# carlostojal/NDT-Net

Hardware: AMD Instinct MI355X
Metric: clouds/sec NDT preprocess+PointNet fwd, 100k pts->1000 NDs, batch=16 (higher is better)
Workload: dtype f64 NDT; PointNet fp32-accurate split-bf16x3 (6 products) on 11 per-point layers, fp32 MFMA on the K=16 first layers and the TNet / seg-bias FC layers

## Files before the change

### include/ndnet_pointnet.h

```cpp
#ifndef NDNET_POINTNET_H_
#define NDNET_POINTNET_H_
#include <stdint.h>

#ifdef __cplusplus
extern "C" {
#endif

#define NDNET_PN_MAX_LAYERS 5

typedef struct ndnet_pn_layer {
  const float* w;
  int64_t w_cloud_stride;
  const float* bias;
  int64_t bias_cloud_stride;
  int32_t K, N;
  int32_t relu;
  int32_t prec;
  int32_t fuse_next;
} ndnet_pn_layer;

typedef struct ndnet_pn_chain {
  const float* x;
  int32_t x_ld;
  int32_t in_cols;
// ... 26 lines not shown
} ndnet_pn_chain;

int ndnet_pn_chain_run(const ndnet_pn_chain *args, int batch, void *stream);
int ndnet_pn_chain_run_t32(const ndnet_pn_chain *args, int batch, void *stream);

int ndnet_pn_debug_stamps(unsigned long long *host, int wgs);
int ndnet_pn_debug_stamps_clear(void);

int ndnet_pn_fc_run(const float *in, int ld_in, const float *W, const float *bias, float *out, int ld_out,
                    int batch, int K, int N, int relu, void *stream);
int ndnet_pn_fc_mfma_run(const float *in, int ld_in, const float *Wf, const float *bias, float *out, int ld_out,
                         int batch, int K, int N, int relu, void *stream);
int ndnet_pn_fc_mfma_bias_run(const float *in, int ld_in, const float *Wf, const float *bias, int bias_ld, float *out,
                              int ld_out, int batch, int K, int N, int relu, void *stream);
int ndnet_pn_cls_head_run(const float *in, int ld_in, const float *Wf, const float *bias, float *probs,
                          int ld_probs, float *logits, int ld_logits, int batch, int K, int N, int out_cols,
                          float *clear, int64_t clear_count, void *stream);
#define NDNET_FOLD_WT 0
#define NDNET_FOLD_FRAG 1
#define NDNET_FOLD_FRAG6 2
#define NDNET_FOLD_ROWS 3
#define NDNET_FOLD_BASIS 4
#define NDNET_FOLD_BIAS 5
typedef struct ndnet_pn_fold_job {
  const float *w;
  const float *bias;
  const float *gamma, *beta, *mean, *var;
  void *out;
  int32_t kind;
  int32_t N, K;
  int32_t ld, k0;
  int32_t Kp, Np;
  int32_t eye;
  float eps;
  int32_t reserved;
  int64_t block0;
} ndnet_pn_fold_job;
int ndnet_pn_fold_prepare(ndnet_pn_fold_job *host_jobs, int num_jobs, int64_t *num_blocks);
int ndnet_pn_fold_run(const ndnet_pn_fold_job *device_jobs, int num_jobs, int64_t num_blocks, void *stream);

int ndnet_pn_head3_run(const float *h2, int ld_h, const float *W3, const float *b3, const float *basis,
                       float *t1, float *w1f, int batch, int K, int kin, int nout, void *stream);

int ndnet_pn_fold_t2_run(const float *w1f, int w1_stride, const float *b1, const float *t2, int t2_ld, float *outf,
                         float *outb, int batch, void *stream);

int ndnet_pn_fold_seg_run(const float *w1f, int w1_stride, const float *b1, const float *t2, int t2_ld, float *outf,
                          float *outb, const float *s1aT, const float *s1b, int N2, float *wd, int64_t wd_stride,
                          float *bd, int64_t bd_stride, int batch, void *stream);

int ndnet_pn_pool12_run(const float *x, int x_ld, int num_points, const float *w0f, int64_t w0_stride,
                        const float *b0, int64_t b0_stride, const float *w_mid, const float *b_mid,
                        const float *w_tail, const float *b_tail, int F, int Fp, float *gmax, int gmax_ld,
                        int batch, void *stream);

#ifdef __cplusplus
}
#endif

#endif
```

### ndt-net_amd/csrc/pointnet_kernels.hip

```cpp
#include <hip/hip_runtime.h>
#include <math.h>
#include <stdint.h>
#include <stdio.h>
#include <stdlib.h>

#include "../../include/ndnet_pointnet.h"

namespace {

#ifndef NDNET_PN_TILE
#define NDNET_PN_TILE 64
#endif
constexpr int kP = NDNET_PN_TILE;
#ifndef NDNET_PN_WAVES
#define NDNET_PN_WAVES (NDNET_PN_TILE / 4)
#endif
constexpr int kWaves = NDNET_PN_WAVES;
constexpr int kThreads = 64 * kWaves;
constexpr int kRowBlocks = kP / 16;
static_assert(kP == 64 || kP == 32, "64- or 32-point tiles");
constexpr int kFuseNC = 64;
constexpr int kPadF = 8;
constexpr int kPadB = 16;
#ifndef NDNET_PN_PLANE_SWZ
// ... 1355 lines not shown
    else bd[(int64_t)b * bd_stride + col] = (float)(acc + (double)sb);
  }
}

#if NDNET_PN_TILE == 64
typedef double f64x4 __attribute__((ext_vector_type(4)));
constexpr int kP12Waves = 16;
constexpr int kP12Pre = 4;
constexpr int kP12Pitch = 130;

__device__ inline void p12_rows(const float* __restrict__ xb, int x_ld, int n, int tile, int kq, int cl, float (&v)[3]) {
  const int p = min(16 * tile + cl, n - 1);
  const float* r = xb + (int64_t)p * x_ld + kq;
#pragma unroll
  for (int s = 0; s < 3; s++) v[s] = r[4 * s];
}

__device__ inline void p12_clean(int n, int tile, int cl, float (&v)[3]) {
  const bool in = 16 * tile + cl < n;
#pragma unroll
  for (int s = 0; s < 3; s++) v[s] = (in & (fabsf(v[s]) < INFINITY)) ? v[s] : NAN;
}

__global__ void __launch_bounds__(kP12Waves * 64) k_pn_pool12(
    const float* __restrict__ x, int x_ld, int n, const float* __restrict__ w0f, int64_t w0_stride,
    const float* __restrict__ b0, int64_t b0_stride, const float* __restrict__ w_mid,
    const float* __restrict__ b_mid, const float* __restrict__ w_tail, const float* __restrict__ b_tail, int Fp,
    float* __restrict__ gmax, int gmax_ld) {
  __shared__ double s_m[13 * kP12Pitch];
  __shared__ float s_wc[13 * 64];
  __shared__ float s_red[kP12Waves * 64];
  const int b = blockIdx.y, c0 = 64 * blockIdx.x;
  const int lane = threadIdx.x & 63, kq = lane >> 4, cl = lane & 15;
  const int wave = __builtin_amdgcn_readfirstlane((int)threadIdx.x >> 6);
  const int tiles = (n + 15) >> 4;
  const float* xb = x + (int64_t)b * n * x_ld;

  float xp[kP12Pre][3];
#pragma unroll
  for (int i = 0; i < kP12Pre; i++) p12_rows(xb, x_ld, n, wave + kP12Waves * i, kq, cl, xp[i]);
  float tw[32];

  if (wave < 8) {
    const float* wb = w0f + (int64_t)b * w0_stride;
    const float* bb = b0 + (int64_t)b * b0_stride;
    float a[16], bw[16];
#pragma unroll
    for (int ks = 0; ks < 16; ks++) {
      const int i = 4 * ks + kq;
      const float* src = cl < 12 ? wb + ((((i >> 4) * 64 + ((cl >> 2) & 3) * 16 + (i & 15)) << 2) + (cl & 3)) : bb + i;
      a[ks] = *src;
      bw[ks] = w_mid[i * 128 + 16 * wave + cl];
    }
#pragma unroll
    for (int ks = 0; ks < 16; ks++) a[ks] = cl < 13 ? a[ks] : 0.0f;
    f64x4 acc0 = {0.0, 0.0, 0.0, 0.0}, acc1 = {0.0, 0.0, 0.0, 0.0};
#pragma unroll
    for (int ks = 0; ks < 16; ks += 2) {
      acc0 = __builtin_amdgcn_mfma_f64_16x16x4f64((double)a[ks], (double)bw[ks], acc0, 0, 0, 0);
      acc1 = __builtin_amdgcn_mfma_f64_16x16x4f64((double)a[ks + 1], (double)bw[ks + 1], acc1, 0, 0, 0);
    }
#pragma unroll
    for (int q = 0; q < 4; q++) {
      const int row = kq + 4 * q, col = 16 * wave + cl;
      double v = acc0[q] + acc1[q];
// ... 1 lines not shown
      if (row < 13) s_m[row * kP12Pitch + col] = v;
    }
  } else if (wave < 12) {
    const int tc = min(c0 + 16 * (wave - 8) + cl, Fp - 1);
#pragma unroll
    for (int ks = 0; ks < 32; ks++) tw[ks] = w_tail[(int64_t)(4 * ks + kq) * Fp + tc];
  }
  __syncthreads();
  if (wave >= 8 && wave < 12) {
    f64x4 acc0 = {0.0, 0.0, 0.0, 0.0}, acc1 = {0.0, 0.0, 0.0, 0.0};
#pragma unroll
    for (int ks = 0; ks < 32; ks += 2) {
      const double a0 = s_m[min(cl, 12) * kP12Pitch + 4 * ks + kq], a1 = s_m[min(cl, 12) * kP12Pitch + 4 * ks + 4 + kq];
      acc0 = __builtin_amdgcn_mfma_f64_16x16x4f64(cl < 13 ? a0 : 0.0, (double)tw[ks], acc0, 0, 0, 0);
      acc1 = __builtin_amdgcn_mfma_f64_16x16x4f64(cl < 13 ? a1 : 0.0, (double)tw[ks + 1], acc1, 0, 0, 0);
    }
#pragma unroll
    for (int q = 0; q < 4; q++) {
      const int row = kq + 4 * q, col = 16 * (wave - 8) + cl;
      double v = acc0[q] + acc1[q];
      if (row == 12) v += (double)b_tail[min(c0 + col, Fp - 1)];
      if (row < 13) s_wc[row * 64 + col] = (float)v;
    }
  }
  __syncthreads();

  float wc[4][3];
#pragma unroll
  for (int cb = 0; cb < 4; cb++)
#pragma unroll
    for (int s = 0; s < 3; s++) wc[cb][s] = s_wc[(4 * s + kq) * 64 + 16 * cb + cl];
  float m[4][4];
#pragma unroll
  for (int cb = 0; cb < 4; cb++)
#pragma unroll
    for (int r = 0; r < 4; r++) m[cb][r] = -INFINITY;
  auto tile = [&](int t, float (&xv)[3]) {
    p12_clean(n, t, cl, xv);
    f32x4 acc[4];
#pragma unroll
    for (int cb = 0; cb < 4; cb++) acc[cb] = f32x4{0.f, 0.f, 0.f, 0.f};
#pragma unroll
    for (int s = 0; s < 3; s++)
#pragma unroll
      for (int cb = 0; cb < 4; cb++) acc[cb] = __builtin_amdgcn_mfma_f32_16x16x4f32(wc[cb][s], xv[s], acc[cb], 0, 0, 0);
#pragma unroll
// ... 101 lines not shown
constexpr int kFoldThreads = 256;

__device__ inline uint16_t fold_bf16(float x) {
  uint32_t u = __float_as_uint(x);
  if ((u & 0x7fffffffu) > 0x7f800000u) return (uint16_t)((u >> 16) | 0x40u);
  return (uint16_t)((u + 0x7fffu + ((u >> 16) & 1u)) >> 16);
}

__device__ inline float fold_w(const ndnet_pn_fold_job& J, int n, int k) {
#pragma clang fp contract(off)
  if (n >= J.N || k >= J.K) return 0.0f;
  const float w = J.w[(int64_t)n * J.ld + J.k0 + k];
  if (!J.gamma) return w;
  return w * (J.gamma[n] / sqrtf(J.var[n] + J.eps));
}

__host__ __device__ inline int64_t fold_units(const ndnet_pn_fold_job& J) {
  switch (J.kind) {
    case NDNET_FOLD_WT: return (int64_t)J.Kp * J.Np;
    case NDNET_FOLD_FRAG: return (int64_t)J.Kp * J.Np / 4;
    case NDNET_FOLD_FRAG6: return (int64_t)J.Kp * J.Np / 8;
    case NDNET_FOLD_ROWS: return (int64_t)J.N * J.K;
    case NDNET_FOLD_BASIS: return (int64_t)9 * J.K * J.N;
    default: return J.Np;
  }
}

__global__ void __launch_bounds__(kFoldThreads) k_pn_fold(const ndnet_pn_fold_job* __restrict__ jobs, int num_jobs) {
#pragma clang fp contract(off)
  int j = 0;
  for (int i = 1; i < num_jobs; i++)
    if (jobs[i].block0 <= (int64_t)blockIdx.x) j = i;
  const ndnet_pn_fold_job J = jobs[j];
  const int64_t u = ((int64_t)blockIdx.x - J.block0) * kFoldThreads + threadIdx.x;
  if (u >= fold_units(J)) return;
  switch (J.kind) {
    case NDNET_FOLD_WT: {
      const int n = (int)(u % J.Np), k = (int)(u / J.Np);
      static_cast<float*>(J.out)[u] = fold_w(J, n, k);
      break;
    }
    case NDNET_FOLD_FRAG: {
      const int kgs = J.Kp / 16;
      const int cl = (int)(u % 16), kq = (int)(u / 16 % 4), kg = (int)(u / 64 % kgs), cb = (int)(u / (64 * kgs));
      const int k = 16 * kg + 4 * kq, n = 16 * cb + cl;
      f32x4 v = {fold_w(J, n, k), fold_w(J, n, k + 1), fold_w(J, n, k + 2), fold_w(J, n, k + 3)};
      reinterpret_cast<f32x4*>(J.out)[u] = v;
      break;
    }
    case NDNET_FOLD_FRAG6: {
      const int kgs = J.Kp / 32;
      const int cl = (int)(u % 16), kq = (int)(u / 16 % 4), kg = (int)(u / 64 % kgs), cb = (int)(u / (64 * kgs));
      const int k = 32 * kg + 8 * kq, n = 16 * cb + cl;
      uint32_t p[3][4];
#pragma unroll
      for (int t = 0; t < 8; t += 2) {
        uint16_t hv[2], mv[2], lv[2];
// ... 10 lines not shown
        p[2][t / 2] = lv[0] | ((uint32_t)lv[1] << 16);
      }
      const int64_t unit = u % 64 + (u / 64) * 192;
      uint4* o = reinterpret_cast<uint4*>(J.out);
#pragma unroll
      for (int pl = 0; pl < 3; pl++) o[unit + 64 * pl] = make_uint4(p[pl][0], p[pl][1], p[pl][2], p[pl][3]);
      break;
    }
    case NDNET_FOLD_ROWS: {
      const int n = (int)(u / J.K), k = (int)(u % J.K);
      static_cast<float*>(J.out)[u] = fold_w(J, n, k);
      break;
    }
    case NDNET_FOLD_BASIS: {
      const int n = (int)(u % J.N), r = (int)(u / J.N % J.K), ac = (int)(u / ((int64_t)J.N * J.K));
      const int a = ac / 3, c = ac % 3;
      float v = 0.0f;
      if (r < 3) {
        if (r == c) v = fold_w(J, n, a);
      } else if ((r - 3) / 3 == c) {
        v = fold_w(J, n, 3 + 3 * a + (r - 3) % 3);
      }
      static_cast<float*>(J.out)[u] = v;
      break;
    }
    default: {
      const int n = (int)u;
      float v = 0.0f;
      if (n < J.N) {
        v = J.bias[n];
        if (J.gamma) v = (v - J.mean[n]) * (J.gamma[n] / sqrtf(J.var[n] + J.eps)) + J.beta[n];
        if (J.eye > 0) v = v + (n / J.eye == n % J.eye ? 1.0f : 0.0f);
      }
      static_cast<float*>(J.out)[u] = v;
    }
  }
}
#endif

#if NDNET_PN_TILE == 64
int fc_mfma_cbw(int nb, int ngmax) {
  static const int cap = [] {
    const char* e = getenv("NDNET_PN_FC_CBW");
    return e ? atoi(e) : 4;
  }();
  for (int c = cap >= 4 ? 4 : cap >= 2 ? 2 : 1; c > 1; c >>= 1)
// ... 76 lines not shown
  k_pn_fold_t2<<<batch, 1024, 0, (hipStream_t)stream>>>(w1f, w1_stride, b1, t2, t2_ld, outf, outb);
  return hipGetLastError() == hipSuccess ? 0 : -21;
}

int ndnet_pn_fold_seg_run(const float* w1f, int w1_stride, const float* b1, const float* t2, int t2_ld, float* outf,
                          float* outb, const float* s1aT, const float* s1b, int N2, float* wd, int64_t wd_stride,
                          float* bd, int64_t bd_stride, int batch, void* stream) {
  if (!w1f || !b1 || !t2 || !outf || !outb || !s1aT || !s1b || !wd || !bd || batch <= 0 || batch > 65535 ||
      w1_stride < 1024 || t2_ld < 4096 || t2_ld % 4 || (uintptr_t)t2 % 16 || N2 <= 0 || N2 % 64 ||
      (uintptr_t)s1aT % 16 || wd_stride < 16 * (int64_t)N2 || bd_stride < N2)
    return -20;
  k_pn_fold_seg<<<dim3(N2 / 64, batch), 1024, 0, (hipStream_t)stream>>>(w1f, w1_stride, b1, t2, t2_ld, outf, outb, s1aT,
                                                                        s1b, N2, wd, wd_stride, bd, bd_stride);
  return hipGetLastError() == hipSuccess ? 0 : -21;
}

int ndnet_pn_pool12_run(const float* x, int x_ld, int num_points, const float* w0f, int64_t w0_stride, const float* b0,
                        int64_t b0_stride, const float* w_mid, const float* b_mid, const float* w_tail,
                        const float* b_tail, int F, int Fp, float* gmax, int gmax_ld, int batch, void* stream) {
  if (!x || !w0f || !b0 || !w_mid || !b_mid || !w_tail || !b_tail || !gmax || batch <= 0 || batch > 65535 ||
      num_points <= 0 || x_ld < 12 || x_ld % 4 || w0_stride < 1024 || b0_stride < 64 || F <= 0 || F > Fp ||
      (Fp != 32 && Fp % 64) || gmax_ld < Fp)
    return -20;
  k_pn_pool12<<<dim3((Fp + 63) / 64, batch), kP12Waves * 64, 0, (hipStream_t)stream>>>(
      x, x_ld, num_points, w0f, w0_stride, b0, b0_stride, w_mid, b_mid, w_tail, b_tail, Fp, gmax, gmax_ld);
  return hipGetLastError() == hipSuccess ? 0 : -21;
}

int ndnet_pn_fold_prepare(ndnet_pn_fold_job* jobs, int num_jobs, int64_t* num_blocks) {
  if (!jobs || num_jobs <= 0 || !num_blocks) return -20;
  int64_t blocks = 0;
  for (int i = 0; i < num_jobs; i++) {
    ndnet_pn_fold_job& J = jobs[i];
    const bool bn = J.gamma != nullptr;
    if (!J.out || (uintptr_t)J.out % 16 || J.kind < NDNET_FOLD_WT || J.kind > NDNET_FOLD_BIAS || J.N <= 0 ||
        (bn && (!J.beta || !J.mean || !J.var || !(J.eps >= 0.0f))) || (!bn && (J.beta || J.mean || J.var)))
      return -20;
    if (J.kind == NDNET_FOLD_BIAS) {
      if (!J.bias || J.Np < J.N || J.eye < 0 || (J.eye > 0 && J.eye * J.eye != J.N)) return -20;
    } else {
      if (!J.w || J.K <= 0 || J.k0 < 0 || J.ld < J.k0 + J.K) return -20;
      if (J.kind == NDNET_FOLD_WT && (J.Kp < J.K || J.Np < J.N)) return -20;
      if (J.kind == NDNET_FOLD_FRAG && (J.Kp < J.K || J.Np < J.N || J.Kp % 16 || J.Np % 16)) return -20;
      if (J.kind == NDNET_FOLD_FRAG6 && (J.Kp < J.K || J.Np < J.N || J.Kp % 32 || J.Np % 16)) return -20;
      if (J.kind == NDNET_FOLD_BASIS && J.K != 12) return -20;
    }
    J.block0 = blocks;
    blocks += (fold_units(J) + kFoldThreads - 1) / kFoldThreads;
  }
  if (blocks <= 0 || blocks > 0x7fffffff) return -20;
  *num_blocks = blocks;
  return 0;
}

int ndnet_pn_fold_run(const ndnet_pn_fold_job* jobs, int num_jobs, int64_t num_blocks, void* stream) {
  if (!jobs || num_jobs <= 0 || num_blocks <= 0 || num_blocks > 0x7fffffff) return -20;
  k_pn_fold<<<(unsigned)num_blocks, kFoldThreads, 0, (hipStream_t)stream>>>(jobs, num_jobs);
  return hipGetLastError() == hipSuccess ? 0 : -21;
}


int ndnet_pn_debug_stamps_clear(void) {
#ifdef NDNET_PN_STAMPS
  static unsigned long long zeros[kStampWgs][16];
  return hipMemcpyToSymbol(HIP_SYMBOL(g_pn_stamps), zeros, sizeof(zeros)) == hipSuccess ? 0 : -21;
#else
  return -20;
#endif
}

int ndnet_pn_debug_stamps(unsigned long long* host, int wgs) {
#ifdef NDNET_PN_STAMPS
  if (!host || wgs <= 0 || wgs > kStampWgs) return -20;
  if (hipDeviceSynchronize() != hipSuccess) return -21;
  return hipMemcpyFromSymbol(host, HIP_SYMBOL(g_pn_stamps), (size_t)wgs * 16 * sizeof(unsigned long long)) ==
                 hipSuccess ? 0 : -21;
#else
  (void)host; (void)wgs;
  return -20;
#endif
// ... 120 lines not shown
```

### ndt-net_amd/ndnet/_lib.py

```python
from __future__ import annotations

import ctypes
import os

import torch

PKG = os.path.dirname(os.path.abspath(__file__))
ROOT = os.path.dirname(PKG)
LIB_PATH = os.environ.get("NDNET_AMD_LIB") or os.path.join(ROOT, "lib", "libndnet_amd.so")

NDNET_OK = 0
NDNET_ERR_ARG = -20
NDNET_ERR_HIP = -21
NDNET_ERR_SYNC = -22
POINT_FILL = {"none": 0, "nearest": 1}
SEG_CONF_LDS_MAX_COLS = 63
FPS_THREADS = 512
FPS_LDS_POINTS = {"float32": 12288, "float64": 6144}
FPS_REG_POINTS = {"float32": 100352, "float64": 49152}


class NdtStats(ctypes.Structure):
    _fields_ = [
        ("rc", ctypes.c_int32),
# ... 119 lines not shown
            fn = getattr(_lib, name)
            fn.restype = res
            fn.argtypes = args
    return _lib


POINTNET_EXPORTS: dict = {
    "ndnet_pn_chain_run": (_I, [_P, _I, _P]),
    "ndnet_pn_chain_run_t32": (_I, [_P, _I, _P]),
    "ndnet_pn_debug_stamps": (_I, [_P, _I]),
    "ndnet_pn_debug_stamps_clear": (_I, []),
    "ndnet_ply_count": (_I, [ctypes.c_char_p, _I, ctypes.POINTER(_U64)]),
    "ndnet_ply_read": (_I, [ctypes.c_char_p, _I, _I, _P, _P, _U64, ctypes.POINTER(_U64), _I]),
    "ndnet_pn_fc_run": (_I, [_P, _I, _P, _P, _P, _I, _I, _I, _I, _I, _P]),
    "ndnet_pn_fc_mfma_run": (_I, [_P, _I, _P, _P, _P, _I, _I, _I, _I, _I, _P]),
    "ndnet_pn_cls_head_run": (_I, [_P, _I, _P, _P, _P, _I, _P, _I, _I, _I, _I, _I, _P, ctypes.c_int64, _P]),
    "ndnet_pn_head3_run": (_I, [_P, _I, _P, _P, _P, _P, _P, _I, _I, _I, _I, _P]),
    "ndnet_pn_fold_t2_run": (_I, [_P, _I, _P, _P, _I, _P, _P, _I, _P]),
    "ndnet_pn_fold_seg_run": (_I, [_P, _I, _P, _P, _I, _P, _P, _P, _P, _I, _P, ctypes.c_int64, _P, ctypes.c_int64, _I,
                                   _P]),
    "ndnet_pn_fc_mfma_bias_run": (_I, [_P, _I, _P, _P, _I, _P, _I, _I, _I, _I, _I, _P]),
    "ndnet_pn_pool12_run": (_I, [_P, _I, _I, _P, ctypes.c_int64, _P, ctypes.c_int64, _P, _P, _P, _P, _I, _I, _P, _I,
                                 _I, _P]),
    "ndnet_pn_fold_prepare": (_I, [_P, _I, ctypes.POINTER(ctypes.c_int64)]),
    "ndnet_pn_fold_run": (_I, [_P, _I, ctypes.c_int64, _P]),
}


_I64 = ctypes.c_int64

TRAIN_EXPORTS: dict = {
    "ndnet_tr_gemm": (_I, [_P, _P, _P, _P, _I64, _I, _I, _I, _I64, _I64, _I64, _I64, _I64, _I64, _I, _I, _I, _I, _I,
                           _I, _P]),
    "ndnet_tr_sum_parts": (_I, [_P, _P, _I64, _I, _P]),
    "ndnet_tr_sum_parts_2d": (_I, [_P, _P, _I64, _I64, _I64, _I, _P]),
    "ndnet_tr_bn_fwd": (_I, [_P, _P, _P, _P, _P, _P, _P, _P, _I, _I, _I, ctypes.c_float, ctypes.c_float, _I, _P, _P,
                             _P, _P]),
    "ndnet_tr_bn_bwd": (_I, [_P, _P, _P, _P, _P, _P, _P, _P, _P, _P, _I, _I, _I, _I, _P, _P]),
    "ndnet_tr_chan_sum": (_I, [_P, _P, _I, _I, _I, _P]),
    "ndnet_tr_row_sum": (_I, [_P, _P, _I64, _I, _P]),
    "ndnet_tr_argmax_match": (_I, [_P, _P, _I64, _I, _P, _P]),
    "ndnet_tr_argmax_match_cm": (_I, [_P, _P, _I, _I, _I, _P, _P, _P]),
    "ndnet_row_argmax": (_I, [_P, _I64, _I, _P, _P]),
    "ndnet_tr_fc_fwd": (_I, [_P, _P, _P, _P, _P, _P, _P, _P, _P, _P, _P, _I, _I, _I, _I64, ctypes.c_float,
                             ctypes.c_float, _I, _I, _P, _P]),
    "ndnet_tr_fc_bwd_w": (_I, [_P, _P, _P, _P, _P, _P, _P, _P, _P, _P, _P, _P, _I, _I, _I, _I64, _I, _P]),
# ... 28 lines not shown
```

### ndt-net_amd/ndnet/models/pointnet_hip.py

```python
from __future__ import annotations

import ctypes
import os

import torch

from .. import _lib

MAX_LAYERS = 5
CHAIN_NAMES = ("A: TNet(3) 3-64-128-1024 + max", "B: conv1(t1) + TNet(64) 64-64-128-1024 + max",
               "C: conv1, conv2(t2), conv3 + max", "D: seg head 64-512-256-128-(C+1) + log_softmax")

chain_timing = None

MODES = {"x6": 1, "fp32": 1, "x3": 2, "bf16": 3}
PRECISION = SPLIT_BF16 = X6_PREC = None


def set_precision(mode: str) -> None:
    global PRECISION, SPLIT_BF16, X6_PREC
    if mode not in MODES:
        raise ValueError(f"unknown PointNet precision mode {mode!r}")
    PRECISION = mode
    SPLIT_BF16 = mode != "fp32"
# ... 38 lines not shown
                ("relu", ctypes.c_int32), ("prec", ctypes.c_int32), ("fuse_next", ctypes.c_int32)]


class _Chain(ctypes.Structure):
    _fields_ = [("x", ctypes.c_void_p), ("x_ld", ctypes.c_int32), ("in_cols", ctypes.c_int32),
                ("num_points", ctypes.c_int32), ("num_layers", ctypes.c_int32), ("L", _Layer * MAX_LAYERS),
                ("mode", ctypes.c_int32), ("out_cols", ctypes.c_int32), ("gmax", ctypes.c_void_p),
                ("gmax_ld", ctypes.c_int32), ("max_width", ctypes.c_int32), ("max_width2", ctypes.c_int32),
                ("out", ctypes.c_void_p), ("clear", ctypes.c_void_p), ("clear_count", ctypes.c_int64),
                ("head_h2", ctypes.c_void_p), ("head_ld", ctypes.c_int32), ("head_K", ctypes.c_int32),
                ("head_w3", ctypes.c_void_p), ("head_b3", ctypes.c_void_p), ("head_basis", ctypes.c_void_p),
                ("head_kin", ctypes.c_int32), ("head_nout", ctypes.c_int32), ("head_t1", ctypes.c_void_p),
                ("fold_t2", ctypes.c_void_p), ("fold_ld", ctypes.c_int32), ("fold_out_w", ctypes.c_void_p),
                ("fold_out_b", ctypes.c_void_p), ("fold_bias", ctypes.c_void_p),
                ("x_nonfinite_nan", ctypes.c_int32), ("reserved0", ctypes.c_int32)]


class _FoldJob(ctypes.Structure):
    _fields_ = [("w", ctypes.c_void_p), ("bias", ctypes.c_void_p), ("gamma", ctypes.c_void_p),
                ("beta", ctypes.c_void_p), ("mean", ctypes.c_void_p), ("var", ctypes.c_void_p),
                ("out", ctypes.c_void_p), ("kind", ctypes.c_int32), ("N", ctypes.c_int32), ("K", ctypes.c_int32),
                ("ld", ctypes.c_int32), ("k0", ctypes.c_int32), ("Kp", ctypes.c_int32), ("Np", ctypes.c_int32),
                ("eye", ctypes.c_int32), ("eps", ctypes.c_float), ("reserved", ctypes.c_int32),
                ("block0", ctypes.c_int64)]



def available() -> bool:
    try:
        return torch.cuda.is_available() and hasattr(_lib.lib(), "ndnet_pn_chain_run")
    except RuntimeError:
        return False


def _pad(n: int, m: int) -> int:
    return (n + m - 1) // m * m


def _bn_fold(w: torch.Tensor, b: torch.Tensor, bn: torch.nn.BatchNorm1d):
    s = bn.weight / torch.sqrt(bn.running_var + bn.eps)
    return w * s[:, None], (b - bn.running_mean) * s + bn.bias


def _wT(w: torch.Tensor, kpad: int, npad: int) -> torch.Tensor:
    n, k = w.shape
    out = torch.zeros((kpad, npad), dtype=torch.float32, device=w.device)
    out[:k, :n] = w.t()
# ... 2 lines not shown

def _frag(wT: torch.Tensor) -> torch.Tensor:
    *lead, K, N = wT.shape
    v = wT.reshape(*lead, K // 16, 4, 4, N // 16, 16)
    nl = len(lead)
    perm = list(range(nl)) + [nl + 3, nl + 0, nl + 1, nl + 4, nl + 2]
    return v.permute(*perm).reshape(*lead, K * N).contiguous()


def _npad(n: int) -> int:
    return 32 if n <= 32 else _pad(n, 64)


def _frag_x6(wT: torch.Tensor) -> torch.Tensor:
    K, N = wT.shape
    w = wT.float()
    h = w.to(torch.bfloat16)
    r = w - h.float()
    m = r.to(torch.bfloat16)
    lo = (r - m.float()).to(torch.bfloat16)
    planes = torch.stack([h, m, lo])
    v = planes.reshape(3, K // 32, 4, 8, N // 16, 16)
    return v.permute(4, 1, 0, 2, 5, 3).reshape(-1).contiguous()


def _bpad(b: torch.Tensor, npad: int) -> torch.Tensor:
    out = torch.zeros(npad, dtype=torch.float32, device=b.device)
    out[: b.shape[0]] = b
    return out


class _Folded:

    def __init__(self, m) -> None:
        fe = m.feature_extractor
        with torch.no_grad():
            def conv(c, bn):
                return _bn_fold(c.weight[:, :, 0].float(), c.bias.float(), bn)

            def tnet(t):
                w1, b1 = conv(t.conv1, t.bn1)
                w2, b2 = conv(t.conv2, t.bn2)
                w3, b3 = conv(t.conv3, t.bn3)
                f1, c1 = _bn_fold(t.fc1.weight.float(), t.fc1.bias.float(), t.bn4)
                f2, c2 = _bn_fold(t.fc2.weight.float(), t.fc2.bias.float(), t.bn5)
                return dict(w1=w1, b1=b1, w2=w2, b2=b2, w3=w3, b3=b3, f1=f1, c1=c1, f2=f2, c2=c2,
                            f3=t.fc3.weight.float(), c3=t.fc3.bias.float())

            self.seg = hasattr(m, "conv4")
            self.baseline = bool(getattr(fe, "points_only", False))
            F = m.feature_dim
            self.F = F
            self.t1 = tnet(fe.t1)
            self.t2 = tnet(fe.t2)
            self.c1w, self.c1b = conv(fe.conv1, fe.bn1)
            self.c2w, self.c2b = conv(fe.conv2, fe.bn2)
            self.c3w, self.c3b = conv(fe.conv3, fe.bn3)
            t1, t2 = self.t1, self.t2
            self.A = [(_wT(t1["w1"], 16, 64), t1["b1"]), (_wT(t1["w2"], 64, 128), t1["b2"]),
                      (_wT(t1["w3"], 128, 1024), t1["b3"])]
            self.B_tail = [(_wT(t2["w1"], 64, 64), t2["b1"]), (_wT(t2["w2"], 64, 128), t2["b2"]),
                           (_wT(t2["w3"], 128, 1024), t2["b3"])]
            self.C_tail = (_wT(self.c3w, 128, _npad(F)), _bpad(self.c3b, _npad(F)))
            self.c1wT = self.c1w.t().contiguous()
            self.C_mid = (_wT(self.c2w, 64, 128), self.c2b)
            dev = self.c1wT.device
            if self.baseline:
                self.t1_basis = None
                self.c1T16 = _wT(self.c1w, 16, 64)
            else:
                E = torch.zeros((9, 12, 12), device=dev)
                for a in range(3):
                    for c in range(3):
                        E[3 * a + c, a, c] = 1.0
                        for j in range(3):
                            E[3 * a + c, 3 + 3 * a + j, 3 + 3 * c + j] = 1.0
                self.t1_basis = torch.matmul(E.transpose(1, 2), self.c1wT).reshape(9, 12 * 64).contiguous()
            self.chain_w = [w for w, _ in self.A + self.B_tail + [self.C_mid, self.C_tail]]
            if self.baseline:
                self.chain_w.append(self.c1T16)
            self.wide = [self.A[2][0], self.B_tail[2][0], self.C_tail[0]]
            self.fcs = [self.t1["f1"], self.t1["f2"], self.t2["f1"], self.t2["f2"], self.t2["f3"]]
            if self.seg:
                self._fold_seg(m, conv)
            else:
                self._fold_cls(m)
            self.wide.append(self.C_mid[0])
            if self.seg:
# ... 107 lines not shown
            add(4, self.t1_basis, fe.conv1, fe.bn1)
        for w in self.chain_w:
            layer, bn, k0, K = src[id(w)]
            add(1, self.frag[id(w)], layer, bn, k0, K, *w.shape)
        for w in self.wide:
            layer, bn, k0, K = src[id(w)]
            add(2, self.frag6[id(w)], layer, bn, k0, K, *w.shape)
        for w in self.fcs:
            layer, bn, k0, K = src[id(w)]
            add(1, self.fcf[id(w)], layer, bn, k0, K, _pad(w.shape[1], 16), w.shape[0])
        if not self.seg:
            add(1, self.h3f, m.conv3, None, 0, 256, 256, self.Cp)
            bias(self.h3b, m.conv3, None)
        return jobs

    def can_refold(self, tensors) -> bool:
        return (self.jobs is not None and self.prec == (X6_NARROW,) and self.c1wT.is_cuda
                and len(tensors) == len(self.tensors) and all(a is b for a, b in zip(tensors, self.tensors))
                and all(t.is_contiguous() and t.dtype == torch.float32 for t in tensors if t.is_floating_point()))

    def refold(self) -> None:
        dev = self.c1wT.device
        if self._dev_jobs is None:
            arr = (_FoldJob * len(self.jobs))()
            for J, (kind, out, layer, bn, k0, K, Kp, Np, eye) in zip(arr, self.jobs):
                J.kind, J.out, J.N, J.K, J.ld, J.k0 = kind, out.data_ptr(), layer.weight.shape[0], K, \
                    layer.weight.shape[1], k0
                J.Kp, J.Np, J.eye = Kp, Np, eye
                if kind == 5:
                    J.bias = layer.bias.data_ptr()
                else:
                    J.w = layer.weight.data_ptr()
                if bn is not None:
                    J.gamma, J.beta = bn.weight.data_ptr(), bn.bias.data_ptr()
                    J.mean, J.var, J.eps = bn.running_mean.data_ptr(), bn.running_var.data_ptr(), bn.eps
            blocks = ctypes.c_int64()
            _lib.check(_lib.lib().ndnet_pn_fold_prepare(arr, len(arr), ctypes.byref(blocks)), "ndnet_pn_fold_prepare")
            self._dev_jobs = torch.frombuffer(bytearray(bytes(arr)), dtype=torch.uint8).to(dev)
            self._blocks = blocks.value
        rc = _lib.lib().ndnet_pn_fold_run(self._dev_jobs.data_ptr(), len(self.jobs), self._blocks,
                                          _lib.stream_ptr(dev))
        _lib.check(rc, "ndnet_pn_fold_run")


def _tensors(m) -> list:
    return list(m.parameters()) + list(m.buffers())


def _signature(tensors) -> tuple:
    return tuple((t.data_ptr(), t._version) for t in tensors)


def _fc_head(g: torch.Tensor, t: dict, dim: int, h1: torch.Tensor, h2: torch.Tensor, out: torch.Tensor):
    torch.addmm(t["c1"], g, t["f1"].t(), out=h1).relu_()
    torch.addmm(t["c2"], h1, t["f2"].t(), out=h2).relu_()
    torch.addmm(t["c3"], h2, t["f3"].t(), out=out)
    return out.view(-1, dim, dim)


def _build_chain(n: int, in_cols: int, layers, relus, mode: int, gmax=None, out_cols=0, fuse=(),
                 x_ld: int = 12) -> "_Chain":
    ch = _Chain()
    ch.x_ld = x_ld
    ch.in_cols = in_cols
# ... 16 lines not shown
            widths[(i + 1) & 1] = max(widths[(i + 1) & 1], N)
    ch.mode = mode
    ch.out_cols = out_cols
    ch.gmax = gmax.data_ptr() if gmax is not None else None
    ch.gmax_ld = gmax.stride(0) if gmax is not None else 0
    ch.max_width, ch.max_width2 = widths
    return ch


TILE32 = os.environ.get("NDNET_PN_TILE32", "1") == "1"
_cus = {}


def _use_t32(B: int, n: int, device) -> bool:
    if not TILE32:
        return False
    if device not in _cus:
        _cus[device] = torch.cuda.get_device_properties(device).multi_processor_count
    return 2 * B * ((n + 63) // 64) <= _cus[device]


class _Pool12:

    def __init__(self, ws: "_Workspace") -> None:
        W = ws.W
        (w_mid, b_mid), (w_tail, b_tail) = W.C_mid, W.C_tail
        assert w_mid.shape == (64, 128) and w_mid.is_contiguous() and w_tail.shape[0] == 128 and w_tail.is_contiguous()
        self.tensors = (ws.w1t2f, ws.b1t2, w_mid, b_mid, w_tail, b_tail, ws.g3)
        self.n, self.F, self.Fp = ws.N, W.F, w_tail.shape[1]
        self.args = (ws.w1t2f.data_ptr(), ws.w1t2f.stride(0), ws.b1t2.data_ptr(), ws.b1t2.stride(0),
                     w_mid.data_ptr(), b_mid.data_ptr(), w_tail.data_ptr(), b_tail.data_ptr(), self.F, self.Fp,
                     ws.g3.data_ptr(), ws.g3.stride(0))


def _run_pool12(blk: "_Pool12", x: torch.Tensor) -> None:
    B, n, _ = x.shape
    assert n == blk.n and x.stride(2) == 1 and x.stride(0) == n * x.stride(1) and x.dtype == torch.float32
    rc = _lib.lib().ndnet_pn_pool12_run(x.data_ptr(), x.stride(1), n, *blk.args, B, _lib.stream_ptr(x.device))
    _lib.check(rc, "ndnet_pn_pool12_run")


def _run_chain(ch, x: torch.Tensor, out=None) -> None:
    if isinstance(ch, _Pool12):
        _run_pool12(ch, x)
        return
    assert x.stride(1) == ch.x_ld and x.stride(2) == 1 and x.dtype == torch.float32
    ch.x = x.data_ptr()
    ch.out = out.data_ptr() if out is not None else None
    if _use_t32(x.shape[0], x.shape[1], x.device):
        rc = _lib.lib().ndnet_pn_chain_run_t32(ctypes.byref(ch), x.shape[0], _lib.stream_ptr(x.device))
        _lib.check(rc, "ndnet_pn_chain_run_t32")
        return
    rc = _lib.lib().ndnet_pn_chain_run(ctypes.byref(ch), x.shape[0], _lib.stream_ptr(x.device))
    _lib.check(rc, "ndnet_pn_chain_run")


def _chain_torch(x: torch.Tensor, n: int, in_cols: int, layers, relus, mode: int, gmax=None, out=None,
                 out_cols=0, fuse=()) -> None:
    h = x[..., :in_cols].float()
    k0 = layers[0][0].shape[-2]
    h = torch.nn.functional.pad(h, (0, k0 - in_cols))
    for i, (w, b) in enumerate(layers):
# ... 31 lines not shown
        self.b1m = None if W.baseline else torch.empty((64,), **f32)
        first = (W.c1T16, W.c1b) if W.baseline else (self.w1T, W.c1b)
        layered = [
            (3, W.A, (1, 1, 1), 0, dict(gmax=self.g1)),
            (kin, [first] + W.B_tail, (0, 1, 1, 1), 0, dict(gmax=self.g2)),
            (kin, [(self.w1t2, self.b1t2), W.C_mid, W.C_tail], (0, 0, 0), 0, dict(gmax=self.g3)),
        ]
        if W.seg:
            layered.append((kin, [(self.w1t2, self.b1t2), (W.s1aT, self.cvec)] + W.D_tail, (0, 1, 1, 1, 0), 1,
                            dict(out_cols=W.C1, fuse=(1,))))
        collapsed = list(layered)
        collapsed[1] = (kin, [(self.w1m, self.b1m)] + W.B_tail[1:], (1, 1, 1), 0, dict(gmax=self.g2))
        self._specs = {(False, False): layered, (True, False): collapsed}
        if W.seg and not W.baseline:
            self.wd = torch.zeros((B, 16 * 512), **f32)
            self.bd = torch.empty((B, 512), **f32)
            self.wdT = torch.empty((B, 12, 512), **f32)
            both = list(collapsed)
            both[3] = (kin, [(self.wdT, self.cvec)] + W.D_tail, (1, 1, 1, 0), 1, dict(out_cols=W.C1, fuse=(0,)))
            self._specs[(True, True)] = both
        self.N = N
        self.structs = {}
        self.pool12 = None

    def collapses_b(self, mode: str = None) -> bool:
        mode = self.mode if mode is None else mode
        return bool(COLLAPSE) and X6_NARROW and not self.W.baseline and mode == "x6"

    def collapses_d(self, mode: str = None) -> bool:
        return (self.collapses_b(mode) and self.W.seg and FOLD_T2_KERNEL and FC_MFMA
                and _npad(self.W.C1) <= COLLAPSE_D_MAX_LAST_N)

    @property
    def specs(self) -> list:
        return self._specs[(self.collapses_b(), self.collapses_d())]

    def uses_pool12(self) -> bool:
        return BACKBONE == "pool12" and FOLD_T2_KERNEL and not self.W.baseline and self.mode in ("x6", "fp32")

    def hip_layers(self, mode: str) -> list:
        W = self.W

        def shared(wb):
            w, b = wb
            if mode != "fp32" and id(w) in W.frag6:
                return (W.frag6[id(w)], 0, b, w.shape[0], w.shape[1], MODES[mode])
            return (W.frag[id(w)], 0, b, w.shape[0], w.shape[1])

        L1 = shared((W.c1T16, W.c1b)) if W.baseline else (self.w1f, self.w1f.stride(0), W.c1b, 16, 64)
        LC = (self.w1t2f, self.w1t2f.stride(0), self.b1t2, 16, 64) if FOLD_T2_KERNEL and not W.baseline else L1
        layers = [
            [shared(x) for x in W.A],
            [L1] + [shared(x) for x in W.B_tail[1 if self.collapses_b(mode) else 0:]],
            [LC, shared(W.C_mid), shared(W.C_tail)],
        ]
        if W.seg and self.collapses_d(mode):
            layers.append([(self.wd, self.wd.stride(0), self.cvec, 16, 512)] + [shared(x) for x in W.D_tail])
        elif W.seg:
            layers.append([(self.w1t2f, self.w1t2f.stride(0), self.b1t2, 16, 64), shared((W.s1aT, self.cvec))] +
                          [shared(x) for x in W.D_tail])
        return layers
# ... 17 lines not shown
            if W.seg:
                structs[3].clear = self.gbuf.data_ptr()
                structs[3].clear_count = self.gbuf.numel()
            if HEAD3_IN_CHAIN and not W.baseline:
                cb = structs[1]
                cb.head_h2, cb.head_ld, cb.head_K = self.h2.data_ptr(), self.h2.stride(0), self.h2.shape[1]
                cb.head_w3, cb.head_b3 = W.t1["f3"].data_ptr(), W.t1["c3"].data_ptr()
                cb.head_basis, cb.head_kin, cb.head_nout = W.t1_basis.data_ptr(), 12, 64
                cb.head_t1 = self.t1.data_ptr()
            if collapse_b:
                cb = structs[1]
                m_w, m_b = W.B_tail[0]
                assert m_w.shape == (64, 64) and m_w.is_contiguous() and m_b.shape == (64,)
                cb.fold_t2, cb.fold_ld, cb.fold_bias = m_w.data_ptr(), 0, m_b.data_ptr()
                cb.x_nonfinite_nan = 1
            if collapse_d:
                structs[3].x_nonfinite_nan = 1
            if not FOLD_T2_KERNEL or W.baseline:
                cc = structs[2]
                cc.fold_t2, cc.fold_ld = self.t2.data_ptr(), self.t2.stride(0)
                cc.fold_out_w, cc.fold_out_b = self.w1t2f.data_ptr(), self.b1t2.data_ptr()
        blk = structs[i]
        if i == 2 and self.uses_pool12():
            if self.pool12 is None:
                self.pool12 = _Pool12(self)
            blk = self.pool12
        if chain_timing is not None:
            e0, e1 = torch.cuda.Event(enable_timing=True), torch.cuda.Event(enable_timing=True)
            e0.record()
            _run_chain(blk, x, out)
            e1.record()
            chain_timing.append((i, e0, e1))
        else:
            _run_chain(blk, x, out)


def _folded(model):
    cache = model._hip
    if cache is None:
        tensors = _tensors(model)
        cache = model._hip = {"tensors": tensors, "sig": None, "stale": False}
    sig = _signature(cache["tensors"])
    cur = _tensors(model)
    replaced = len(cur) != len(cache["tensors"]) or any(a is not b for a, b in zip(cur, cache["tensors"]))
    if replaced or cache["sig"] != sig or cache["stale"]:
        W = cache.get("W")
        if W is not None and W.can_refold(_tensors(model)):
            W.refold()
        else:
            cache.update(tensors=_tensors(model), W=_Folded(model), ws={})
            sig = _signature(cache["tensors"])
        cache.update(sig=sig, stale=False)
    return cache


FOLD_T2_KERNEL = os.environ.get("NDNET_PN_FOLD_T2", "kernel") == "kernel"
BACKBONE = os.environ.get("NDNET_PN_BACKBONE", "pool12")
if BACKBONE not in ("pool12", "chain"):
    raise ValueError(f"NDNET_PN_BACKBONE must be 'pool12' or 'chain', not {BACKBONE!r}")
COLLAPSE = os.environ.get("NDNET_PN_COLLAPSE", "1") == "1"
HEAD3_IN_CHAIN = os.environ.get("NDNET_PN_HEAD3", "chain") == "chain"

FC_MFMA = os.environ.get("NDNET_PN_FC", "mfma") == "mfma"


def _fc(x: torch.Tensor, w: torch.Tensor, b: torch.Tensor, out: torch.Tensor, relu: bool, wf=None) -> None:
    B = x.shape[0]
    st = _lib.stream_ptr(x.device)
    for c0 in range(0, B, 16):
        n = min(16, B - c0)
        if FC_MFMA and wf is not None:
            rc = _lib.lib().ndnet_pn_fc_mfma_run(x[c0].data_ptr(), x.stride(0), wf.data_ptr(), b.data_ptr(),
                                                 out[c0].data_ptr(), out.stride(0), n, _pad(w.shape[1], 16),
                                                 w.shape[0], 1 if relu else 0, st)
            _lib.check(rc, "ndnet_pn_fc_mfma_run")
        else:
            rc = _lib.lib().ndnet_pn_fc_run(x[c0].data_ptr(), x.stride(0), w.data_ptr(), b.data_ptr(),
                                            out[c0].data_ptr(), out.stride(0), n, w.shape[1], w.shape[0],
                                            1 if relu else 0, st)
            _lib.check(rc, "ndnet_pn_fc_run")


def _glue_hip(W, ws, B: int):
# ... 168 lines not shown
```

Before: 91400.

## Pre-fold mid and tail weight matrices into one f64 product for pool12

Computes the product of the mid (64x128) and tail (128xF) weights in f64 once at fold time, together with a combined bias. The pool12 kernel then builds its per-cloud 13xF collapsed weight with a single 64-deep f64 MFMA pass on four waves. This replaces the two-stage 64->128->F computation and its shared-memory staging. The fold launcher is split so the product jobs run as a separate launch after the other fold jobs they depend on, which adds a launch and a serial f64 dot-product kernel.

```diff
diff --git a/include/ndnet_pointnet.h b/include/ndnet_pointnet.h
--- a/include/ndnet_pointnet.h
+++ b/include/ndnet_pointnet.h
@@ -72,6 +72,7 @@
 #define NDNET_FOLD_ROWS 3
 #define NDNET_FOLD_BASIS 4
 #define NDNET_FOLD_BIAS 5
+#define NDNET_FOLD_PROD 6
 typedef struct ndnet_pn_fold_job {
   const float *w;
   const float *bias;
@@ -85,6 +86,9 @@
   float eps;
   int32_t reserved;
   int64_t block0;
+  const float *rhs;
+  int32_t out_f64;
+  int32_t reserved1;
 } ndnet_pn_fold_job;
 int ndnet_pn_fold_prepare(ndnet_pn_fold_job *host_jobs, int num_jobs, int64_t *num_blocks);
 int ndnet_pn_fold_run(const ndnet_pn_fold_job *device_jobs, int num_jobs, int64_t num_blocks, void *stream);
@@ -104,6 +108,10 @@
                         const float *w_tail, const float *b_tail, int F, int Fp, float *gmax, int gmax_ld,
                         int batch, void *stream);
 
+int ndnet_pn_pool12_tail_run(const float *x, int x_ld, int num_points, const float *w0f, int64_t w0_stride,
+                             const float *b0, int64_t b0_stride, const double *w23, const double *b23, int Fp,
+                             float *gmax, int gmax_ld, int batch, void *stream);
+
 #ifdef __cplusplus
 }
 #endif
diff --git a/ndt-net_amd/csrc/pointnet_kernels.hip b/ndt-net_amd/csrc/pointnet_kernels.hip
--- a/ndt-net_amd/csrc/pointnet_kernels.hip
+++ b/ndt-net_amd/csrc/pointnet_kernels.hip
@@ -1401,12 +1401,13 @@
   for (int s = 0; s < 3; s++) v[s] = (in & (fabsf(v[s]) < INFINITY)) ? v[s] : NAN;
 }
 
+template <bool kTail>
 __global__ void __launch_bounds__(kP12Waves * 64) k_pn_pool12(
     const float* __restrict__ x, int x_ld, int n, const float* __restrict__ w0f, int64_t w0_stride,
     const float* __restrict__ b0, int64_t b0_stride, const float* __restrict__ w_mid,
-    const float* __restrict__ b_mid, const float* __restrict__ w_tail, const float* __restrict__ b_tail, int Fp,
-    float* __restrict__ gmax, int gmax_ld) {
-  __shared__ double s_m[13 * kP12Pitch];
+    const float* __restrict__ b_mid, const float* __restrict__ w_tail, const float* __restrict__ b_tail,
+    const double* __restrict__ w23, const double* __restrict__ b23, int Fp, float* __restrict__ gmax, int gmax_ld) {
+  __shared__ double s_m[kTail ? 1 : 13 * kP12Pitch];
   __shared__ float s_wc[13 * 64];
   __shared__ float s_red[kP12Waves * 64];
   const int b = blockIdx.y, c0 = 64 * blockIdx.x;
@@ -1420,6 +1421,38 @@
   for (int i = 0; i < kP12Pre; i++) p12_rows(xb, x_ld, n, wave + kP12Waves * i, kq, cl, xp[i]);
   float tw[32];
 
+  if constexpr (kTail) {
+    if (wave < 4) {
+      const float* wb = w0f + (int64_t)b * w0_stride;
+      const float* bb = b0 + (int64_t)b * b0_stride;
+      const int tc = min(c0 + 16 * wave + cl, Fp - 1);
+      float a[16];
+      double bw[16];
+#pragma unroll
+      for (int ks = 0; ks < 16; ks++) {
+        const int i = 4 * ks + kq;
+        const float* src = cl < 12 ? wb + ((((i >> 4) * 64 + ((cl >> 2) & 3) * 16 + (i & 15)) << 2) + (cl & 3)) : bb + i;
+        a[ks] = *src;
+        bw[ks] = w23[(int64_t)i * Fp + tc];
+      }
+      const double brow = b23[tc];
+#pragma unroll
+      for (int ks = 0; ks < 16; ks++) a[ks] = cl < 13 ? a[ks] : 0.0f;
+      f64x4 acc[4];
+#pragma unroll
+      for (int j = 0; j < 4; j++) acc[j] = f64x4{0.0, 0.0, 0.0, 0.0};
+#pragma unroll
+      for (int ks = 0; ks < 16; ks++)
+        acc[ks & 3] = __builtin_amdgcn_mfma_f64_16x16x4f64((double)a[ks], bw[ks], acc[ks & 3], 0, 0, 0);
+#pragma unroll
+      for (int q = 0; q < 4; q++) {
+        const int row = kq + 4 * q, col = 16 * wave + cl;
+        double v = (acc[0][q] + acc[1][q]) + (acc[2][q] + acc[3][q]);
+        if (row == 12) v += brow;
+        if (row < 13) s_wc[row * 64 + col] = (float)v;
+      }
+    }
+  } else {
   if (wave < 8) {
     const float* wb = w0f + (int64_t)b * w0_stride;
     const float* bb = b0 + (int64_t)b * b0_stride;
@@ -1467,6 +1500,7 @@
       if (row == 12) v += (double)b_tail[min(c0 + col, Fp - 1)];
       if (row < 13) s_wc[row * 64 + col] = (float)v;
     }
+  }
   }
   __syncthreads();
 
@@ -1614,17 +1648,20 @@
     case NDNET_FOLD_FRAG6: return (int64_t)J.Kp * J.Np / 8;
     case NDNET_FOLD_ROWS: return (int64_t)J.N * J.K;
     case NDNET_FOLD_BASIS: return (int64_t)9 * J.K * J.N;
+    case NDNET_FOLD_PROD: return (int64_t)J.N * J.Np;
     default: return J.Np;
   }
 }
 
-__global__ void __launch_bounds__(kFoldThreads) k_pn_fold(const ndnet_pn_fold_job* __restrict__ jobs, int num_jobs) {
+__global__ void __launch_bounds__(kFoldThreads) k_pn_fold(const ndnet_pn_fold_job* __restrict__ jobs, int num_jobs,
+                                                          int64_t block_base) {
 #pragma clang fp contract(off)
+  const int64_t blk = block_base + blockIdx.x;
   int j = 0;
   for (int i = 1; i < num_jobs; i++)
-    if (jobs[i].block0 <= (int64_t)blockIdx.x) j = i;
+    if (jobs[i].block0 <= blk) j = i;
   const ndnet_pn_fold_job J = jobs[j];
-  const int64_t u = ((int64_t)blockIdx.x - J.block0) * kFoldThreads + threadIdx.x;
+  const int64_t u = (blk - J.block0) * kFoldThreads + threadIdx.x;
   if (u >= fold_units(J)) return;
   switch (J.kind) {
     case NDNET_FOLD_WT: {
@@ -1681,6 +1718,16 @@
         v = fold_w(J, n, 3 + 3 * a + (r - 3) % 3);
       }
       static_cast<float*>(J.out)[u] = v;
+      break;
+    }
+    case NDNET_FOLD_PROD: {
+      const int n = (int)(u % J.Np), r = (int)(u / J.Np);
+      const float* a = J.w + (int64_t)r * J.ld + J.k0;
+      double acc = 0.0;
+      for (int k = 0; k < J.K; k++) acc += (double)a[k] * (double)J.rhs[(int64_t)k * J.Np + n];
+      if (J.bias) acc += (double)J.bias[n];
+      if (J.out_f64) static_cast<double*>(J.out)[u] = acc;
+      else static_cast<float*>(J.out)[u] = (float)acc;
       break;
     }
     default: {
@@ -1803,18 +1850,38 @@
       num_points <= 0 || x_ld < 12 || x_ld % 4 || w0_stride < 1024 || b0_stride < 64 || F <= 0 || F > Fp ||
       (Fp != 32 && Fp % 64) || gmax_ld < Fp)
     return -20;
-  k_pn_pool12<<<dim3((Fp + 63) / 64, batch), kP12Waves * 64, 0, (hipStream_t)stream>>>(
-      x, x_ld, num_points, w0f, w0_stride, b0, b0_stride, w_mid, b_mid, w_tail, b_tail, Fp, gmax, gmax_ld);
+  k_pn_pool12<false><<<dim3((Fp + 63) / 64, batch), kP12Waves * 64, 0, (hipStream_t)stream>>>(
+      x, x_ld, num_points, w0f, w0_stride, b0, b0_stride, w_mid, b_mid, w_tail, b_tail, nullptr, nullptr, Fp, gmax,
+      gmax_ld);
+  return hipGetLastError() == hipSuccess ? 0 : -21;
+}
+
+int ndnet_pn_pool12_tail_run(const float* x, int x_ld, int num_points, const float* w0f, int64_t w0_stride,
+                             const float* b0, int64_t b0_stride, const double* w23, const double* b23, int Fp,
+                             float* gmax, int gmax_ld, int batch, void* stream) {
+  if (!x || !w0f || !b0 || !w23 || !b23 || !gmax || batch <= 0 || batch > 65535 || num_points <= 0 || x_ld < 12 ||
+      x_ld % 4 || w0_stride < 1024 || b0_stride < 64 || Fp <= 0 || (Fp != 32 && Fp % 64) || gmax_ld < Fp ||
+      ((uintptr_t)w23 | (uintptr_t)b23) % 8)
+    return -20;
+  k_pn_pool12<true><<<dim3((Fp + 63) / 64, batch), kP12Waves * 64, 0, (hipStream_t)stream>>>(
+      x, x_ld, num_points, w0f, w0_stride, b0, b0_stride, nullptr, nullptr, nullptr, nullptr, w23, b23, Fp, gmax,
+      gmax_ld);
   return hipGetLastError() == hipSuccess ? 0 : -21;
 }
 
 int ndnet_pn_fold_prepare(ndnet_pn_fold_job* jobs, int num_jobs, int64_t* num_blocks) {
   if (!jobs || num_jobs <= 0 || !num_blocks) return -20;
-  int64_t blocks = 0;
+  int64_t blocks = 0, prod0 = -1;
   for (int i = 0; i < num_jobs; i++) {
     ndnet_pn_fold_job& J = jobs[i];
     const bool bn = J.gamma != nullptr;
-    if (!J.out || (uintptr_t)J.out % 16 || J.kind < NDNET_FOLD_WT || J.kind > NDNET_FOLD_BIAS || J.N <= 0 ||
+    if (J.kind == NDNET_FOLD_PROD) {
+      if (bn || !J.rhs || J.Np <= 0 || (J.out_f64 != 0 && J.out_f64 != 1)) return -20;
+      if (prod0 < 0) prod0 = blocks;
+    } else if (prod0 >= 0) {
+      return -20;
+    }
+    if (!J.out || (uintptr_t)J.out % 16 || J.kind < NDNET_FOLD_WT || J.kind > NDNET_FOLD_PROD || J.N <= 0 ||
         (bn && (!J.beta || !J.mean || !J.var || !(J.eps >= 0.0f))) || (!bn && (J.beta || J.mean || J.var)))
       return -20;
     if (J.kind == NDNET_FOLD_BIAS) {
@@ -1830,13 +1897,15 @@
     blocks += (fold_units(J) + kFoldThreads - 1) / kFoldThreads;
   }
   if (blocks <= 0 || blocks > 0x7fffffff) return -20;
-  *num_blocks = blocks;
+  *num_blocks = blocks | ((prod0 < 0 ? 0 : blocks - prod0) << 32);
   return 0;
 }
 
 int ndnet_pn_fold_run(const ndnet_pn_fold_job* jobs, int num_jobs, int64_t num_blocks, void* stream) {
-  if (!jobs || num_jobs <= 0 || num_blocks <= 0 || num_blocks > 0x7fffffff) return -20;
-  k_pn_fold<<<(unsigned)num_blocks, kFoldThreads, 0, (hipStream_t)stream>>>(jobs, num_jobs);
+  const int64_t blocks = num_blocks & 0xffffffff, prod = num_blocks >> 32;
+  if (!jobs || num_jobs <= 0 || blocks <= 0 || blocks > 0x7fffffff || prod < 0 || prod > blocks) return -20;
+  if (blocks > prod) k_pn_fold<<<(unsigned)(blocks - prod), kFoldThreads, 0, (hipStream_t)stream>>>(jobs, num_jobs, 0);
+  if (prod) k_pn_fold<<<(unsigned)prod, kFoldThreads, 0, (hipStream_t)stream>>>(jobs, num_jobs, blocks - prod);
   return hipGetLastError() == hipSuccess ? 0 : -21;
 }
 
diff --git a/ndt-net_amd/ndnet/_lib.py b/ndt-net_amd/ndnet/_lib.py
--- a/ndt-net_amd/ndnet/_lib.py
+++ b/ndt-net_amd/ndnet/_lib.py
@@ -165,6 +165,7 @@
     "ndnet_pn_fc_mfma_bias_run": (_I, [_P, _I, _P, _P, _I, _P, _I, _I, _I, _I, _I, _P]),
     "ndnet_pn_pool12_run": (_I, [_P, _I, _I, _P, ctypes.c_int64, _P, ctypes.c_int64, _P, _P, _P, _P, _I, _I, _P, _I,
                                  _I, _P]),
+    "ndnet_pn_pool12_tail_run": (_I, [_P, _I, _I, _P, ctypes.c_int64, _P, ctypes.c_int64, _P, _P, _I, _P, _I, _I, _P]),
     "ndnet_pn_fold_prepare": (_I, [_P, _I, ctypes.POINTER(ctypes.c_int64)]),
     "ndnet_pn_fold_run": (_I, [_P, _I, ctypes.c_int64, _P]),
 }
diff --git a/ndt-net_amd/ndnet/models/pointnet_hip.py b/ndt-net_amd/ndnet/models/pointnet_hip.py
--- a/ndt-net_amd/ndnet/models/pointnet_hip.py
+++ b/ndt-net_amd/ndnet/models/pointnet_hip.py
@@ -84,7 +84,8 @@
                 ("out", ctypes.c_void_p), ("kind", ctypes.c_int32), ("N", ctypes.c_int32), ("K", ctypes.c_int32),
                 ("ld", ctypes.c_int32), ("k0", ctypes.c_int32), ("Kp", ctypes.c_int32), ("Np", ctypes.c_int32),
                 ("eye", ctypes.c_int32), ("eps", ctypes.c_float), ("reserved", ctypes.c_int32),
-                ("block0", ctypes.c_int64)]
+                ("block0", ctypes.c_int64), ("rhs", ctypes.c_void_p), ("out_f64", ctypes.c_int32),
+                ("reserved1", ctypes.c_int32)]
 
 
 
@@ -133,6 +134,14 @@
     planes = torch.stack([h, m, lo])
     v = planes.reshape(3, K // 32, 4, 8, N // 16, 16)
     return v.permute(4, 1, 0, 2, 5, 3).reshape(-1).contiguous()
+
+
+def _prod64(a: torch.Tensor, rhs: torch.Tensor, bias=None) -> torch.Tensor:
+    a, rhs = a.reshape(-1, a.shape[-1]).double(), rhs.double()
+    acc = torch.zeros((a.shape[0], rhs.shape[1]), dtype=torch.float64, device=a.device)
+    for k in range(a.shape[1]):
+        acc += a[:, k, None] * rhs[k]
+    return acc if bias is None else acc + bias.double()
 
 
 def _bpad(b: torch.Tensor, npad: int) -> torch.Tensor:
@@ -174,7 +183,13 @@
                            (_wT(t2["w3"], 128, 1024), t2["b3"])]
             self.C_tail = (_wT(self.c3w, 128, _npad(F)), _bpad(self.c3b, _npad(F)))
             self.c1wT = self.c1w.t().contiguous()
+            self.products = []
             self.C_mid = (_wT(self.c2w, 64, 128), self.c2b)
+            if not self.baseline:
+                self.W23 = _prod64(self.C_mid[0], self.C_tail[0])
+                self.b23 = _prod64(self.c2b[None, :], self.C_tail[0], self.C_tail[1]).reshape(-1)
+                self.products += [(self.W23, self.C_mid[0], self.C_tail[0], None),
+                                  (self.b23, self.c2b, self.C_tail[0], self.C_tail[1])]
             dev = self.c1wT.device
             if self.baseline:
                 self.t1_basis = None
@@ -328,7 +343,16 @@
     def refold(self) -> None:
         dev = self.c1wT.device
         if self._dev_jobs is None:
-            arr = (_FoldJob * len(self.jobs))()
+            arr = (_FoldJob * (len(self.jobs) + len(self.products)))()
+            for i, (out, a, rhs, bias) in enumerate(self.products, len(self.jobs)):
+                J = arr[i]
+                assert a.is_contiguous() and rhs.is_contiguous() and rhs.dim() == 2 and out.is_contiguous()
+                J.kind, J.out, J.w, J.rhs = 6, out.data_ptr(), a.data_ptr(), rhs.data_ptr()
+                J.K, J.ld, J.Np = rhs.shape[0], rhs.shape[0], rhs.shape[1]
+                J.N = a.numel() // J.K
+                J.bias = bias.data_ptr() if bias is not None else None
+                J.out_f64 = 1 if out.dtype == torch.float64 else 0
+                assert out.numel() == J.N * J.Np
             for J, (kind, out, layer, bn, k0, K, Kp, Np, eye) in zip(arr, self.jobs):
                 J.kind, J.out, J.N, J.K, J.ld, J.k0 = kind, out.data_ptr(), layer.weight.shape[0], K, \
                     layer.weight.shape[1], k0
@@ -344,8 +368,8 @@
             _lib.check(_lib.lib().ndnet_pn_fold_prepare(arr, len(arr), ctypes.byref(blocks)), "ndnet_pn_fold_prepare")
             self._dev_jobs = torch.frombuffer(bytearray(bytes(arr)), dtype=torch.uint8).to(dev)
             self._blocks = blocks.value
-        rc = _lib.lib().ndnet_pn_fold_run(self._dev_jobs.data_ptr(), len(self.jobs), self._blocks,
-                                          _lib.stream_ptr(dev))
+        rc = _lib.lib().ndnet_pn_fold_run(self._dev_jobs.data_ptr(), len(self.jobs) + len(self.products),
+                                          self._blocks, _lib.stream_ptr(dev))
         _lib.check(rc, "ndnet_pn_fold_run")
 
 
@@ -408,22 +432,29 @@
 
 class _Pool12:
 
-    def __init__(self, ws: "_Workspace") -> None:
+    def __init__(self, ws: "_Workspace", tail: bool = False) -> None:
         W = ws.W
         (w_mid, b_mid), (w_tail, b_tail) = W.C_mid, W.C_tail
         assert w_mid.shape == (64, 128) and w_mid.is_contiguous() and w_tail.shape[0] == 128 and w_tail.is_contiguous()
+        self.n, self.F, self.Fp = ws.N, W.F, w_tail.shape[1]
+        self.tail = tail
+        head = (ws.w1t2f.data_ptr(), ws.w1t2f.stride(0), ws.b1t2.data_ptr(), ws.b1t2.stride(0))
+        if tail:
+            assert W.W23.shape == (64, self.Fp) and W.W23.dtype == W.b23.dtype == torch.float64
+            self.tensors = (ws.w1t2f, ws.b1t2, W.W23, W.b23, ws.g3)
+            self.args = head + (W.W23.data_ptr(), W.b23.data_ptr(), self.Fp, ws.g3.data_ptr(), ws.g3.stride(0))
+            return
         self.tensors = (ws.w1t2f, ws.b1t2, w_mid, b_mid, w_tail, b_tail, ws.g3)
-        self.n, self.F, self.Fp = ws.N, W.F, w_tail.shape[1]
-        self.args = (ws.w1t2f.data_ptr(), ws.w1t2f.stride(0), ws.b1t2.data_ptr(), ws.b1t2.stride(0),
-                     w_mid.data_ptr(), b_mid.data_ptr(), w_tail.data_ptr(), b_tail.data_ptr(), self.F, self.Fp,
-                     ws.g3.data_ptr(), ws.g3.stride(0))
+        self.args = head + (w_mid.data_ptr(), b_mid.data_ptr(), w_tail.data_ptr(), b_tail.data_ptr(), self.F, self.Fp,
+                            ws.g3.data_ptr(), ws.g3.stride(0))
 
 
 def _run_pool12(blk: "_Pool12", x: torch.Tensor) -> None:
     B, n, _ = x.shape
     assert n == blk.n and x.stride(2) == 1 and x.stride(0) == n * x.stride(1) and x.dtype == torch.float32
-    rc = _lib.lib().ndnet_pn_pool12_run(x.data_ptr(), x.stride(1), n, *blk.args, B, _lib.stream_ptr(x.device))
-    _lib.check(rc, "ndnet_pn_pool12_run")
+    name = "ndnet_pn_pool12_tail_run" if blk.tail else "ndnet_pn_pool12_run"
+    rc = getattr(_lib.lib(), name)(x.data_ptr(), x.stride(1), n, *blk.args, B, _lib.stream_ptr(x.device))
+    _lib.check(rc, name)
 
 
 def _run_chain(ch, x: torch.Tensor, out=None) -> None:
@@ -501,6 +532,7 @@
         self.N = N
         self.structs = {}
         self.pool12 = None
+        self._pool12 = {}
 
     def collapses_b(self, mode: str = None) -> bool:
         mode = self.mode if mode is None else mode
@@ -516,6 +548,9 @@
 
     def uses_pool12(self) -> bool:
         return BACKBONE == "pool12" and FOLD_T2_KERNEL and not self.W.baseline and self.mode in ("x6", "fp32")
+
+    def uses_tail(self) -> bool:
+        return bool(FOLD_PRODUCTS) and bool(COLLAPSE) and self.uses_pool12()
 
     def hip_layers(self, mode: str) -> list:
         W = self.W
@@ -579,9 +614,10 @@
                 cc.fold_out_w, cc.fold_out_b = self.w1t2f.data_ptr(), self.b1t2.data_ptr()
         blk = structs[i]
         if i == 2 and self.uses_pool12():
-            if self.pool12 is None:
-                self.pool12 = _Pool12(self)
-            blk = self.pool12
+            tail = self.uses_tail()
+            if tail not in self._pool12:
+                self._pool12[tail] = _Pool12(self, tail)
+            blk = self.pool12 = self._pool12[tail]
         if chain_timing is not None:
             e0, e1 = torch.cuda.Event(enable_timing=True), torch.cuda.Event(enable_timing=True)
             e0.record()
@@ -616,6 +652,7 @@
 if BACKBONE not in ("pool12", "chain"):
     raise ValueError(f"NDNET_PN_BACKBONE must be 'pool12' or 'chain', not {BACKBONE!r}")
 COLLAPSE = os.environ.get("NDNET_PN_COLLAPSE", "1") == "1"
+FOLD_PRODUCTS = os.environ.get("NDNET_PN_FOLD_PRODUCTS", "1") == "1"
 HEAD3_IN_CHAIN = os.environ.get("NDNET_PN_HEAD3", "chain") == "chain"
 
 FC_MFMA = os.environ.get("NDNET_PN_FC", "mfma") == "mfma"
```

Result: faster. 93640 (median of 6 runs) (+2.5%).
